# koide3/hdl_graph_slam

Hardware: AMD Instinct MI355X
Metric: registrations/sec (64-beam ~120k-pt pair), loop-closure batch (higher is better)
Workload: dtype f64; 1 GPU; loop-closure batch: 64 candidate keyframes/GPU x HDL-64E (~118849 pts) vs 1 query keyframe, FAST_GICP + getFitnessScore, cold (index + covariances rebuilt every step); candidate set: SURVEY 8d (distinct ray-casts at poses within 20 m of the query, guess = ground truth + 0.5 m / 2 deg noise, z forced to 0); candidates_per_gpu=64, points_per_cloud=118849, method=FAST_GICP, distinct_scans=16, parallelism=single GPU

## Files before the change

### hdl_graph_slam_amd/csrc/hgs_bvh.h

```cpp
#pragma once
#include "hgs_math.h"

namespace hgs {

constexpr int kLeaf = 8;

#if defined(__HIPCC__)
typedef float4 Float4;
#else
struct alignas(16) Float4 {
  float x, y, z, w;
};
#endif

struct BvhView {
  const Float4* nodes;
  const Float4* pts;
  const Float4* lpts;
  int P;
  int n;
};

HGS_HD void bvh_load_box(const Float4* nodes, uint32_t n, float* mn, float* mx) {
  const float* g = reinterpret_cast<const float*>(nodes) + 32 * (size_t)(n >> 2) + (n & 3u);
// ... 166 lines not shown
```

### hdl_graph_slam_amd/csrc/hgs_consts.h

```cpp
#pragma once
#include <cfloat>
#include <cmath>

#include "../../include/hgs_registration.h"
#include "hgs_floor.h"
#include "hgs_gicp.h"
#include "hgs_icp.h"
#include "hgs_ndt.h"
#include "hgs_vgicp.h"

namespace hgs {

inline GicpConsts gicp_consts(const hgs_params& p) {
  GicpConsts c;
  const double thr = p.max_correspondence_distance;
  c.max_corr2 = thr * thr;
  c.search_bound2 = c.max_corr2 >= (double)FLT_MAX ? FLT_MAX : nextafterf((float)c.max_corr2, FLT_MAX);
  c.rotation_eps = p.rotation_epsilon;
  c.translation_eps = p.transformation_epsilon;
  c.lm_init_lambda_factor = p.lm_init_lambda_factor;
  c.lm_max_iterations = p.lm_max_iterations;
  c.max_iterations = p.max_iterations;
  c.k_correspondences = p.correspondence_randomness;
  return c;
}

inline VgicpConsts vgicp_consts(const hgs_params& p) {
  VgicpConsts c;
  c.resolution = p.resolution;
  c.search = p.neighbor_search == HGS_DIRECT27 ? 3 : (p.neighbor_search == HGS_DIRECT7 ? 2 : 1);
  c.pad = 0;
  return c;
}

inline IcpConsts icp_consts(const hgs_params& p) {
  IcpConsts c;
  const double thr = p.max_correspondence_distance;
  c.max_corr2 = thr * thr;
  c.search_bound2 = c.max_corr2 >= (double)FLT_MAX ? FLT_MAX : nextafterf((float)c.max_corr2, FLT_MAX);
  c.max_iterations = p.max_iterations;
  c.trans_eps = p.transformation_epsilon;
  c.rot_thr = p.rotation_epsilon > 0 ? p.rotation_epsilon : 1.0 - p.transformation_epsilon;
  c.reciprocal = p.icp_reciprocal ? 1 : 0;
  c.pad = 0;
  return c;
}

inline NdtConsts ndt_consts(const hgs_params& p) {
  NdtConsts c;
  const double c1 = 10.0 * (1 - p.ndt_outlier_ratio);
  const double c2 = p.ndt_outlier_ratio / std::pow(p.resolution, 3);
  const double d3 = -std::log(c2);
  c.gauss_d1 = -std::log(c1 + c2) - d3;
  c.gauss_d2 = -2 * std::log((-std::log(c1 * std::exp(-0.5) + c2) - d3) / c.gauss_d1);
  c.step_size = p.ndt_step_size;
  c.trans_eps = p.transformation_epsilon;
  c.max_iterations = p.max_iterations;
  c.search = p.neighbor_search == HGS_DIRECT1 ? 1 : (p.neighbor_search == HGS_KDTREE ? 0 : 2);
  c.kdtree_radius2 = (float)(p.resolution * p.resolution);
// ... 24 lines not shown
```

### hdl_graph_slam_amd/csrc/hgs_device.h

```cpp
#pragma once
#include <hip/hip_runtime.h>
#include "hgs_gicp.h"
#include "hgs_floor.h"
#include "hgs_icp.h"
#include "hgs_ndt.h"
#include "hgs_vgicp.h"

namespace hgs {

struct CloudMeta {
  int nvalid;
  int ndt_ncells;
  unsigned bbmin[3];
  unsigned bbmax[3];
  int ndt_min_b[3], ndt_max_b[3], ndt_div_mul[3];
  int ndt_error;
  int vg_ncells;
  int vg_min_b[3], vg_max_b[3], vg_div_mul[3];
  int vg_error;
  int pad[1];
};

struct CloudDesc {
  const float4* raw;
// ... 68 lines not shown
void launch_hilbert_keys(hipStream_t s, const CloudDesc* descs, int ncloud, int max_n, unsigned long long* keys, unsigned* vals, int drop_bits);
void launch_gather_sorted(hipStream_t s, const CloudDesc* descs, int ncloud, int max_slots, const unsigned* sorted_vals);
void launch_build_tree(hipStream_t s, const CloudDesc* descs, int ncloud, int max_P);
void launch_knn_cov(hipStream_t s, const CloudDesc* descs, int ncloud, int max_n, int k, int qpw, int reg_method, int gather ,
                    double* raw_stage = nullptr );

void launch_gicp_init(hipStream_t s, GicpState* states, const float* guesses, int B, Progress prog);
struct Guess16 {
  float m[16];
};
void launch_gicp_init1(hipStream_t s, GicpState* states, const float* guess_host , Progress prog);
void launch_gicp_linearize(hipStream_t s, const CloudDesc* descs, TargetView tgt, const GicpState* states, GicpConsts c, double* partials, int max_blocks, int B,
                           int qpw);
void launch_gicp_solve(hipStream_t s, const CloudDesc* descs, GicpState* states, GicpConsts c, const double* partials, int max_blocks, int B,
                       int tile_points );
void launch_gicp_error(hipStream_t s, const CloudDesc* descs, TargetView tgt, const GicpState* states, double* partials_err, int max_blocks, int B);
void launch_gicp_linearize_round2(hipStream_t s, const CloudDesc* descs, TargetView tgt, const GicpState* states_in, GicpState* states_out, GicpConsts c, double* partials,
                                  const double* partials_err, int max_blocks , int lin_blocks , int B, int qpw, Progress prog,
                                  DevResult* results, DevResult* early_out );
void launch_gicp_error_round2(hipStream_t s, const CloudDesc* descs, TargetView tgt, const GicpState* states_in, GicpState* states_out, GicpConsts c, const double* partials,
                              double* partials_err, int max_blocks, int err_blocks , int B, int lin_tile_points);
void launch_gicp_decide(hipStream_t s, const CloudDesc* descs, GicpState* states, GicpConsts c, const double* partials_err, int max_blocks, int B, Progress prog);
void launch_gicp_results(hipStream_t s, const GicpState* states, DevResult* out, int B);

void launch_icp_init(hipStream_t s, IcpState* states, const float* guesses, int B, Progress prog);
void launch_icp_correspond(hipStream_t s, const CloudDesc* descs, TargetView tgt, const IcpState* states, IcpConsts c, double* partials, int max_blocks, int B);
void launch_icp_solve(hipStream_t s, const CloudDesc* descs, IcpState* states, IcpConsts c, const double* partials, int max_blocks, int B, Progress prog);
void launch_icp_results(hipStream_t s, const IcpState* states, DevResult* out, int B);

void launch_fitness(hipStream_t s, const CloudDesc* descs, TargetView tgt, const DevResult* poses, double max_range, double* partials, int max_blocks, int B,
                    int use_seed, int qpw);
void launch_fitness_final(hipStream_t s, const CloudDesc* descs, const double* partials, int max_blocks, DevResult* out, int B, int tile_pts);
void launch_gicp_linearize(hipStream_t s, const CloudDesc* descs, const TargetView* tviews, const GicpState* states, GicpConsts c, double* partials, int max_blocks, int B,
                           int qpw);
void launch_gicp_error(hipStream_t s, const CloudDesc* descs, const TargetView* tviews, const GicpState* states, double* partials_err, int max_blocks, int B);
void launch_gicp_linearize_round2(hipStream_t s, const CloudDesc* descs, const TargetView* tviews, const GicpState* states_in, GicpState* states_out, GicpConsts c, double* partials,
                                  const double* partials_err, int max_blocks, int lin_blocks, int B, int qpw, Progress prog, DevResult* results, DevResult* early_out);
void launch_gicp_error_round2(hipStream_t s, const CloudDesc* descs, const TargetView* tviews, const GicpState* states_in, GicpState* states_out, GicpConsts c, const double* partials,
                              double* partials_err, int max_blocks, int err_blocks, int B, int lin_tile_points);
void launch_icp_correspond(hipStream_t s, const CloudDesc* descs, const TargetView* tviews, const IcpState* states, IcpConsts c, double* partials, int max_blocks, int B);
void launch_fitness(hipStream_t s, const CloudDesc* descs, const TargetView* tviews, const DevResult* poses, double max_range, double* partials, int max_blocks, int B,
                    int use_seed, int qpw);
}
struct hgs_result;
namespace hgs {
void launch_results_to_records(hipStream_t s, const DevResult* res, const int* candidate_ids, int n, int n_slots, ::hgs_result* out);
void launch_nn_query(hipStream_t s, TargetView tgt, const float4* q, int nq, int* idx, float* d2);
void launch_seed_grid_build(hipStream_t s, const float4* pts, const CloudMeta* meta, int n_max, unsigned* tab, int bits);
inline size_t seed_grid_entries(int bits) { return ((size_t)1 << bits) + ((size_t)1 << (bits - 2)) + ((size_t)1 << (bits - 4)); }
void launch_transform(hipStream_t s, const float4* raw, int n, const float* T16_colmajor_dev, float4* out);
// ... 90 lines not shown
```

### hdl_graph_slam_amd/csrc/hgs_engine.hip

```cpp
#include <hip/hip_runtime.h>
#include <algorithm>
#include <atomic>
#include <chrono>
#include <climits>
#include <condition_variable>
#include <cmath>
#include <cstdio>
#include <cstdlib>
#include <cstring>
#include <exception>
#include <limits>
#include <mutex>
#include <new>
#include <stdexcept>
#include <string>
#include <thread>
#include <vector>

#include "../../include/hgs_registration.h"
#include "hgs_comm.h"
#include "hgs_consts.h"
#include "hgs_device.h"
#include "hgs_resources.h"
#include "hgs_sort.h"
// ... 67 lines not shown
  int prefilter_fast = 1;
  int upload_trace = 0;
  int floor_chunk = 64;
  int early_run_ahead = 2;
  int early_result = 1;
  PinnedBuffer h_early;
  hipEvent_t early_event = nullptr;
  bool early_pending = false, early_valid = false;
  int fused_rounds = 1;
  int fused_rounds_below = 262144;
  int fused_rounds_max_problems = kFusedRoundMaxProblems, fused_rounds_max_blocks = 640;
  int cov_split = 1;
  int resident_descs = 1;
  int knn_qpw_tiny = -1;
  int knn_tiny_below = 32768;
  int seed_grid = 1;
  int knn_replay = -1;
  int batch_lanes = 0;
  std::string err;
  hgs_cloud* target = nullptr;
  hgs_cloud* source = nullptr;
  bool own_target = false, own_source = false;
  float final_T[16];

  DeviceBuffer staging, sort_keys[2], sort_vals[2], sort_tmp, descs, states, angles, partials, partials_err, results, guesses, done, misc;
  DeviceBuffer lane_partials[7], lane_partials_err[7];
  DeviceBuffer ndt_accum;
  DeviceBuffer group_tviews, group_corr;
  hgs::Comm* comm = nullptr;
  DeviceBuffer comm_send, comm_recv, comm_ids;
// ... 637 lines not shown
  return upload_descs(h, sources, false, &s.d_descs, nullptr, corr_of);
}

bool corr_seeds_fitness(int method) { return method == HGS_FAST_GICP || method == HGS_ICP; }
void lane_fitness(hgs_handle* h, BatchLane& L, const BatchShape& s, double max_range, bool corr_seeds) {
  StageTimer tm(h, HGS_STAGE_FITNESS);
  DevResult* res = h->results.as<DevResult>() + L.b0;
  with_lane_target(s, L, s.d_tviews ? TargetView{} : target_view(h->target),
                   [&](auto tgt) { launch_fitness(L.stream, s.d_descs + L.b0, tgt, res, max_range, L.partials_err, s.max_blocks, L.B, corr_seeds ? 1 : 0, s.qpw); });
  launch_fitness_final(L.stream, s.d_descs + L.b0, L.partials_err, s.max_blocks, res, L.B, s.nn_tile);
}
void lane_fitness_tail(hgs_handle* h, BatchLane& L, const BatchShape& s, const double* fit_max_range) {
  if (fit_max_range) lane_fitness(h, L, s, *fit_max_range, corr_seeds_fitness(h->prm.method));
}

int run_gicp_rounds(hgs_handle* h, const BatchShape& s, const float* guesses_host, bool guess_in_args, const double* fit_max_range) {
  const int B = s.B, max_blocks = s.max_blocks;
  hgs_cloud* tgt = h->target;
  const bool voxel = h->prm.method == HGS_FAST_VGICP;
  const GicpConsts c = gicp_consts(h->prm);
  const VgicpConsts vc = vgicp_consts(h->prm);
  const bool round2 = s.gicp_round2;
  const bool early = round2 && B == 1 && !fit_max_range && h->early_result && !h->profiling;
  DevResult* early_out = nullptr;
  if (early) {
    HGS_HIP(h, h->h_early.reserve(sizeof(DevResult)));
    early_out = h->h_early.as<DevResult>();
  }
  HGS_HIP(h, h->states.reserve((size_t)B * sizeof(GicpState) * (round2 ? 2 : 1)));
  GicpState* st = h->states.as<GicpState>();
  GicpState* st_other = st + B;
  const TargetView tv = s.d_tviews ? TargetView{} : target_view(tgt);
  const NdtTargetView vtv = voxel ? vgicp_target_view(tgt) : NdtTargetView{};
  const long max_rounds = (long)std::max(1, c.max_iterations) * std::max(1, c.lm_max_iterations) + 2 + (round2 ? 1 : 0);
  std::vector<BatchLane> lanes;
// ... 26 lines not shown
      });
      return;
    }
    {
      StageTimer tm(h, HGS_STAGE_LINEARIZE);
      if (voxel) launch_vgicp_linearize(L.stream, dd, vtv, ls, vc, L.partials, max_blocks, L.B);
      else with_lane_target(s, L, tv, [&](auto t) { launch_gicp_linearize(L.stream, dd, t, ls, c, L.partials, max_blocks, L.B, s.qpw); });
    }
    {
      StageTimer tm(h, HGS_STAGE_SOLVE);
      launch_gicp_solve(L.stream, dd, ls, c, L.partials, max_blocks, L.B, voxel ? kBlock : s.nn_tile);
    }
    {
      StageTimer tm(h, HGS_STAGE_ERROR);
      if (voxel) launch_vgicp_error(L.stream, dd, vtv, ls, vc, L.partials_err, max_blocks, L.B);
      else with_lane_target(s, L, tv, [&](auto t) { launch_gicp_error(L.stream, dd, t, ls, L.partials_err, max_blocks, L.B); });
    }
    {
      StageTimer tm(h, HGS_STAGE_SOLVE);
      launch_gicp_decide(L.stream, dd, ls, c, L.partials_err, max_blocks, L.B, L.prog);
    }
  }, finish_lane, early ? (long)h->early_run_ahead : kRunAhead);
  HGS_TRY(close_lanes(h, lanes));
  if (h->early_valid) {
    if (!h->early_event) HGS_HIP(h, hipEventCreateWithFlags(&h->early_event, hipEventDisableTiming));
    HGS_HIP(h, hipEventRecord(h->early_event, h->stream));
    h->early_pending = true;
  }
  return HGS_OK;
}

int run_icp_rounds(hgs_handle* h, const BatchShape& s, const double* fit_max_range) {
  const int B = s.B, max_blocks = s.max_blocks;
  const IcpConsts c = icp_consts(h->prm);
  HGS_HIP(h, h->states.reserve((size_t)B * sizeof(IcpState)));
  IcpState* st = h->states.as<IcpState>();
  const TargetView tv = s.d_tviews ? TargetView{} : target_view(h->target);
  const long max_rounds = (long)std::max(0, c.max_iterations) + 2;
  std::vector<BatchLane> lanes;
  HGS_TRY(open_lanes(h, B, (size_t)max_blocks * kAccIcp * sizeof(double), (size_t)max_blocks * 2 * sizeof(double), lanes, s.err_blocks));
  auto finish_lane = [&](BatchLane& L) {
    launch_icp_results(L.stream, st + L.b0, h->results.as<DevResult>() + L.b0, L.B);
    lane_fitness_tail(h, L, s, fit_max_range);
  };
  for (BatchLane& L : lanes) launch_icp_init(L.stream, st + L.b0, h->guesses.as<float>() + (size_t)L.b0 * 16, L.B, L.prog);
  drive_lanes(lanes, max_rounds, [&](BatchLane& L) {
    {
      StageTimer tm(h, HGS_STAGE_LINEARIZE);
      with_lane_target(s, L, tv, [&](auto t) { launch_icp_correspond(L.stream, s.d_descs + L.b0, t, st + L.b0, c, L.partials, max_blocks, L.B); });
// ... 274 lines not shown
  const std::string k(key);
  if (k == "batch_lanes") h->batch_lanes = value <= 0 ? 0 : std::min(kMaxLanes, value);
  else if (k == "lane_start") h->lane_start = value != 0 ? 1 : 0;
  else if (k == "ndt_sort") h->ndt_sort = std::max(-1, std::min(1, value));
  else if (k == "cov_split") h->cov_split = value != 0 ? 1 : 0;
  else if (k == "fused_rounds") h->fused_rounds = value != 0 ? 1 : 0;
  else if (k == "early_result") h->early_result = value != 0 ? 1 : 0;
  else if (k == "early_run_ahead") h->early_run_ahead = std::max(1, std::min(8, value));
  else if (k == "fused_rounds_max_problems") h->fused_rounds_max_problems = std::max(0, value);
  else if (k == "fused_rounds_max_blocks") h->fused_rounds_max_blocks = std::max(0, value);
  else if (k == "fused_rounds_below") h->fused_rounds_below = std::max(0, value);
  else if (k == "resident_descs") h->resident_descs = value != 0 ? 1 : 0;
  else if (k == "knn_qpw_tiny") h->knn_qpw_tiny = value < 0 ? -1 : std::max(0, std::min(32, value & ~7));
  else if (k == "knn_tiny_below") h->knn_tiny_below = std::max(0, value);
  else if (k == "seed_grid") h->seed_grid = value != 0 ? 1 : 0;
  else if (k == "knn_replay") h->knn_replay = std::max(-1, std::min(2, value));
  else if (k == "ndt_resident") h->ndt_resident_blocks = std::max(0, value);
  else if (k == "ndt_chunk") h->ndt_chunk = std::max(0, value);
  else if (k == "hilbert_levels") h->hilbert_levels = std::max(4, std::min(16, value));
  else if (k == "nn_qpw") h->nn_qpw = value == 16 ? 16 : (value == 32 ? 32 : (value == 64 ? 64 : 0));
  else if (k == "nn_qpw16_below") h->nn_qpw16_below = std::max(0, value);
  else if (k == "nn_qpw32_below") h->nn_qpw32_below = std::max(0, value);
  else if (k == "upload_trace") h->upload_trace = value != 0 ? 1 : 0;
  else if (k == "prefilter_fast") h->prefilter_fast = value != 0 ? 1 : 0;
  else if (k == "floor_chunk") h->floor_chunk = std::max(1, std::min(kFloorMaxChunk, value));
  else {
    h->err = "hgs_debug_set_option: unknown option '" + k + "'";
    return HGS_ERR_INVALID_ARGUMENT;
  }
  return HGS_OK;
// ... 1278 lines not shown
  const bool voxel = h->prm.method == HGS_FAST_VGICP;
  std::vector<hgs_cloud*> all{s, t};
  HGS_TRY(ensure_cov(h, all, h->prm.correspondence_randomness));
  if (voxel) HGS_TRY(ensure_vgicp_target(h, t));
  const int max_blocks = std::max(1, ((int)s->n_input + kBlock - 1) / kBlock);
  std::vector<hgs_cloud*> src{s};
  const CloudDesc* d_descs = nullptr;
  HGS_TRY(upload_descs(h, src, false, &d_descs, nullptr));
  HGS_HIP(h, h->states.reserve(sizeof(GicpState)));
  HGS_HIP(h, h->partials.reserve((size_t)max_blocks * kAcc * sizeof(double)));
  HGS_HIP(h, h->misc.reserve(64 * sizeof(double)));
  HGS_HIP(h, hipMemsetAsync(h->partials.p, 0, (size_t)max_blocks * kAcc * sizeof(double), h->stream));
  HGS_HIP(h, hipMemcpyAsync(h->misc.p, T12, 12 * sizeof(double), hipMemcpyHostToDevice, h->stream));
  launch_gicp_debug_state(h->stream, h->states.as<GicpState>(), h->misc.as<double>());
  if (voxel) launch_vgicp_linearize(h->stream, d_descs, vgicp_target_view(t), h->states.as<GicpState>(), vgicp_consts(h->prm), h->partials.as<double>(), max_blocks, 1);
  else launch_gicp_linearize(h->stream, d_descs, target_view(t), h->states.as<GicpState>(), gicp_consts(h->prm), h->partials.as<double>(), max_blocks, 1, 64);
  double* d_out = h->misc.as<double>() + 16;
  launch_reduce_partials(h->stream, h->partials.as<double>(), max_blocks, kAcc, d_out);
  double acc[kAcc];
  HGS_HIP(h, hipMemcpyAsync(acc, d_out, sizeof(acc), hipMemcpyDeviceToHost, h->stream));
  const size_t s_slots = (size_t)s->P * kLeaf, t_slots = (size_t)t->P * kLeaf;
  std::vector<float4> spts, tpts;
  std::vector<int> dcorr;
  int s_nvalid = 0;
  if (corr) {
    spts.resize(s_slots), tpts.resize(t_slots), dcorr.resize(s_slots);
    HGS_HIP(h, hipMemcpyAsync(spts.data(), s->desc.pts, s_slots * sizeof(float4), hipMemcpyDeviceToHost, h->stream));
    HGS_HIP(h, hipMemcpyAsync(tpts.data(), t->desc.pts, t_slots * sizeof(float4), hipMemcpyDeviceToHost, h->stream));
    HGS_HIP(h, hipMemcpyAsync(dcorr.data(), s->desc.corr, s_slots * sizeof(int), hipMemcpyDeviceToHost, h->stream));
    HGS_HIP(h, hipMemcpyAsync(&s_nvalid, &s->desc.meta->nvalid, sizeof(int), hipMemcpyDeviceToHost, h->stream));
  }
// ... 27 lines not shown
  if (!h->source) return HGS_ERR_NO_SOURCE;
  HGS_TRY(set_device(h));
  hgs_cloud *s = h->source, *t = h->target;
  std::vector<hgs_cloud*> all{s, t};
  HGS_TRY(ensure_index(h, all));
  const int max_blocks = std::max(1, ((int)s->n_input + kTileNN - 1) / kTileNN);
  std::vector<hgs_cloud*> src{s};
  const CloudDesc* d_descs = nullptr;
  HGS_TRY(upload_descs(h, src, false, &d_descs, nullptr));
  IcpState st;
  for (int i = 0; i < 12; i++) st.x.m[i] = T12[i];
  st.mse = st.mse_prev = DBL_MAX, st.phase = ICP_RUN, st.iterations = st.passes = st.converged = 0;
  HGS_HIP(h, h->states.reserve(sizeof(IcpState)));
  HGS_HIP(h, h->partials.reserve((size_t)max_blocks * kAccIcp * sizeof(double)));
  HGS_HIP(h, hipMemcpyAsync(h->states.p, &st, sizeof(st), hipMemcpyHostToDevice, h->stream));
  launch_icp_correspond(h->stream, d_descs, target_view(t), h->states.as<IcpState>(), icp_consts(h->prm), h->partials.as<double>(), max_blocks, 1);
  HGS_HIP(h, hipGetLastError());
  std::vector<double> part((size_t)max_blocks * kAccIcp);
  int s_nvalid = 0;
  HGS_HIP(h, hipMemcpyAsync(&s_nvalid, &s->desc.meta->nvalid, sizeof(int), hipMemcpyDeviceToHost, h->stream));
  HGS_HIP(h, hipMemcpyAsync(part.data(), h->partials.p, part.size() * sizeof(double), hipMemcpyDeviceToHost, h->stream));
  const size_t s_slots = (size_t)s->P * kLeaf, t_slots = (size_t)t->P * kLeaf;
  std::vector<float4> spts, tpts;
  std::vector<int> dcorr;
  if (corr) {
    spts.resize(s_slots), tpts.resize(t_slots), dcorr.resize(s_slots);
    HGS_HIP(h, hipMemcpyAsync(spts.data(), s->desc.pts, s_slots * sizeof(float4), hipMemcpyDeviceToHost, h->stream));
    HGS_HIP(h, hipMemcpyAsync(tpts.data(), t->desc.pts, t_slots * sizeof(float4), hipMemcpyDeviceToHost, h->stream));
    HGS_HIP(h, hipMemcpyAsync(dcorr.data(), s->desc.corr, s_slots * sizeof(int), hipMemcpyDeviceToHost, h->stream));
  }
  HGS_HIP(h, hipStreamSynchronize(h->stream));
// ... 137 lines not shown
```

### hdl_graph_slam_amd/csrc/hgs_gicp.h

```cpp
#pragma once
#include "hgs_bvh.h"

namespace hgs {

constexpr int kAcc = 28;

struct GicpConsts {
  double max_corr2;
  float search_bound2;
  double rotation_eps, translation_eps;
  double lm_init_lambda_factor;
  int lm_max_iterations;
  int max_iterations;
  int k_correspondences;
};

HGS_HD Sym3 gicp_neighbour_cov(const double* s1, const Sym3& s2, int found, int k, double lambda) {
  const double inv_f = 1.0 / (double)found, inv_k = 1.0 / (double)k;
  const double mx = s1[0] * inv_f, my = s1[1] * inv_f, mz = s1[2] * inv_f;
  Sym3 c;
  c.xx = (s2.xx - found * mx * mx) * inv_k + lambda;
  c.xy = (s2.xy - found * mx * my) * inv_k;
  c.xz = (s2.xz - found * mx * mz) * inv_k;
  c.yy = (s2.yy - found * my * my) * inv_k + lambda;
  c.yz = (s2.yz - found * my * mz) * inv_k;
  c.zz = (s2.zz - found * mz * mz) * inv_k + lambda;
  return c;
}
HGS_HD Sym3 gicp_regularized_cov(const double* s1, const Sym3& s2, int found, int k) {
// ... 252 lines not shown
```

### hdl_graph_slam_amd/csrc/hgs_icp.h

```cpp
#pragma once
#include "hgs_math.h"

namespace hgs {

constexpr int kAccIcp = 17;

struct IcpConsts {
  double max_corr2;
  float search_bound2;
  int max_iterations;
  double trans_eps;
  double rot_thr;
  int reciprocal;
  int pad;
};

enum IcpPhase { ICP_RUN = 0, ICP_DONE = 2 };

struct IcpState {
  Pose x;
  double mse;
  double mse_prev;
  int phase;
  int iterations;
  int passes;
  int converged;
};

HGS_HD void icp_state_init(IcpState& s, const float* guess_colmajor) {
// ... 148 lines not shown
```

### hdl_graph_slam_amd/csrc/hgs_kernels.hip

```cpp
#include <hip/hip_runtime.h>
#include "../../include/hgs_registration.h"
#include "hgs_device.h"
#include "hgs_wave_bvh.h"

namespace hgs {

#ifndef HGS_OPAQUE_POINTER
#define HGS_OPAQUE_POINTER(p) asm volatile("" : "+v"(p))
#define HGS_WAIT_VMEM() asm volatile("s_waitcnt vmcnt(0)" ::: "memory")
#define HGS_LANE_ID(dst) asm volatile("v_mbcnt_lo_u32_b32 %0, -1, 0\n\tv_mbcnt_hi_u32_b32 %0, -1, %0" : "=v"(dst))
#endif
#ifndef HGS_COMPILER_MEMORY_BARRIER
#define HGS_COMPILER_MEMORY_BARRIER() asm volatile("" ::: "memory")
#endif
#ifndef HGS_LOAD_GLOBAL_XYZ
__device__ __forceinline__ float4 hgs_load_global_xyz(const float4* p) {
  const __attribute__((address_space(1))) float* g = (const __attribute__((address_space(1))) float*)(p);
  return make_float4(g[0], g[1], g[2], 0.f);
}
#define HGS_LOAD_GLOBAL_XYZ(p) hgs_load_global_xyz(p)
#define HGS_OPAQUE_OFFSET(off) asm volatile("" : "+v"(off))
#define HGS_WAIT_VMEM_TRACKED() __builtin_amdgcn_s_waitcnt(0x0F70)
#endif
#ifndef HGS_LINEARIZE_WAVES
// ... 287 lines not shown
}
void launch_hilbert_keys(hipStream_t s, const CloudDesc* descs, int ncloud, int max_n, unsigned long long* keys, unsigned* vals, int drop_bits) {
  if (max_n <= 0) return;
  hipLaunchKernelGGL(k_hilbert_keys, dim3((max_n + kBlock - 1) / kBlock, ncloud), dim3(kBlock), 0, s, descs, keys, vals, drop_bits);
}

__global__ __launch_bounds__(kBlock) void k_gather_sorted(const CloudDesc* descs, const unsigned* __restrict__ sorted_vals) {
  const CloudDesc d = descs[blockIdx.y];
  const int i = blockIdx.x * kBlock + threadIdx.x;
  if (i >= d.P * kLeaf) return;
  float4 p = make_float4(INFINITY, INFINITY, INFINITY, __int_as_float(-1));
  if (i < d.meta->nvalid) p = d.raw[sorted_vals[d.sort_off + i]];
  d.pts[i] = p;
  float* leaf = reinterpret_cast<float*>(d.lpts) + 32 * (size_t)(i >> 3) + (i & 7);
  leaf[0] = p.x, leaf[8] = p.y, leaf[16] = p.z, leaf[24] = p.w;
  if (d.pad) d.corr[i] = -1;
}
void launch_gather_sorted(hipStream_t s, const CloudDesc* descs, int ncloud, int max_slots, const unsigned* sorted_vals) {
  if (max_slots <= 0) return;
  hipLaunchKernelGGL(k_gather_sorted, dim3((max_slots + kBlock - 1) / kBlock, ncloud), dim3(kBlock), 0, s, descs, sorted_vals);
}

__device__ __forceinline__ void store_walk_sentinels(float4* nodes) {
  const float mn[3] = {INFINITY, INFINITY, INFINITY}, mx[3] = {-INFINITY, -INFINITY, -INFINITY};
  bvh_store_box(nodes, 0u, mn, mx);
  bvh_store_box(nodes, 1u, mn, mx);
}

__global__ __launch_bounds__(kBlock) void k_build_bottom(const CloudDesc* descs) {
  const CloudDesc d = descs[blockIdx.y];
  const int P = d.P;
// ... 356 lines not shown
  const unsigned n = (unsigned)t.meta->nvalid;
  int best = -1;
  float best_d = FLT_MAX;
  const unsigned e[3] = {e0, e1, e2};
#pragma unroll
  for (int l = 0; l < 3; l++) {
    if (e[l] < n) {
      const float4 p = t.pts[e[l]];
      const float d = dist2f(q, p.x, p.y, p.z);
      if (d < best_d) best_d = d, best = (int)e[l];
    }
  }
  return best;
}

__device__ __forceinline__ void packet_nn1(const BvhView& tv, float* park, const F3& q, bool active, float bound2, int seed, int qpw, float& d2, int& pos, int& orig) {
  const bool seeded = seed >= 0 && seed < tv.n;
  int leaf;
  bool tie, found;
  if (__ballot(active && !seeded) != 0ull) wave_nn1_quad<true, true>(tv, park, q, active, bound2, seed, qpw >> 1, d2, leaf, tie, found);
  else wave_nn1_quad<false, true>(tv, park, q, active, bound2, seed, qpw >> 1, d2, leaf, tie, found);
  if (__ballot(tie) != 0ull) {
    const F3 qa[1] = {q};
    const bool aa[1] = {active};
    const int sa[1] = {seed};
    float da[1];
    int pa[1], oa[1];
    wave_nn1<1>(tv, park, qa, aa, bound2, sa, da, pa, oa, qpw);
    d2 = da[0], pos = pa[0], orig = oa[0];
  } else {
    nn1_resolve_leaf(tv, q, found ? leaf : -1, d2, pos, orig);
  }
// ... 27 lines not shown
  {
    double t[kAcc];
    gicp_point_terms_by_slot(r, M, t);
#pragma unroll
    for (int j = 0; j < 14; j++) even[j] = t[2 * j];
  }
  __builtin_amdgcn_sched_barrier(0);
  {
    double t[kAcc];
    gicp_point_terms_by_slot(r, M, t);
#pragma unroll
    for (int j = 0; j < 14; j++) odd[j] = t[2 * j + 1];
  }
  wave_sums28_to(even, odd, row, lane);
}

template <bool ROUND2, bool SHORT = false, typename TGT = TargetView>
__global__ __launch_bounds__(kBlock) __attribute__((amdgpu_waves_per_eu(ROUND2 ? 4 : HGS_LINEARIZE_WAVES))) void k_gicp_linearize(const CloudDesc* descs, TGT tgt_arg, const GicpState* states, GicpConsts c,
                                                           double* __restrict__ partials, int max_blocks, int qpw, GicpState* states_out,
                                                           const double* __restrict__ partials_err, Progress prog, DevResult* results, DevResult* early_out) {
  const int b = blockIdx.y;
  const TargetView& tgt = problem_target(tgt_arg, b);
  __shared__ GicpState st2;
  __shared__ double ws2[kGicpControlWorkspace];
  if constexpr (!ROUND2) {
    if (states[b].phase != GICP_LINEARIZE) return;
  }
  const CloudDesc d = descs[b];
  const int n = d.meta->nvalid;
  if constexpr (ROUND2) {
// ... 29 lines not shown
  if (tile >= ntiles) return;
  __shared__ double lds[4 * kAcc];
  __shared__ unsigned arrivals;
  __shared__ __attribute__((aligned(512))) float park[kBlock / 64][kParkFloats];
  if (threadIdx.x == 0) arrivals = 0u;
  __syncthreads();
  const int wave = __builtin_amdgcn_readfirstlane((int)(threadIdx.x >> 6));
  const Pose T = ROUND2 ? st2.x0 : states[b].x0;
  float Tf[12];
  pose_to_float(T, Tf);
  static_assert(kNW == 1, "one packet of 64 consecutive source points per wave");
  const int idx = tile * tile_pts + wave * qpw + (int)(threadIdx.x & 63);
  const bool active = (int)(threadIdx.x & 63) < qpw && idx < n;
  const float4 a = active ? load_stream(d.pts + idx) : make_float4(0.f, 0.f, 0.f, 0.f);
  const F3 q = transform_point_f(Tf, a.x, a.y, a.z);
  const int seed = active ? __builtin_nontemporal_load(d.corr + idx) : -1;
  float d2;
  int j, orig;
  packet_nn1(view_of(tgt), park[wave], q, active, c.search_bound2, seed, qpw, d2, j, orig);
  const double R[9] = {T.m[0], T.m[1], T.m[2], T.m[4], T.m[5], T.m[6], T.m[8], T.m[9], T.m[10]};
  int jj = active ? j : -1;
  if (jj >= 0 && !((double)d2 < c.max_corr2)) jj = -1;
  if (active) __builtin_nontemporal_store(jj, d.corr + idx);
  if constexpr (SHORT) {
    static_assert(ROUND2, "the short-packet form belongs to the two-launch rounds");
    {
      __shared__ int chunk_corr[kBlock];
      int lane;
      HGS_LANE_ID(lane);
      if (lane < qpw) chunk_corr[wave * qpw + lane] = jj;
      unsigned ticket = 0;
      if (lane == 0) ticket = __hip_atomic_fetch_add(&arrivals, 1u, __ATOMIC_ACQ_REL, __HIP_MEMORY_SCOPE_WORKGROUP);
      ticket = (unsigned)__builtin_amdgcn_readlane((int)ticket, 0);
      if (ticket != kBlock / 64 - 1) return;
      const int chunks = tile_pts / 64;
      for (int ch = 0; ch < chunks; ch++) {
        const int i2 = tile * tile_pts + ch * 64 + lane;
        if (tile * tile_pts + ch * 64 >= n) break;
        const int j2 = i2 < n ? chunk_corr[ch * 64 + lane] : -1;
        Sym3 M2 = {0.0, 0.0, 0.0, 0.0, 0.0, 0.0};
        GicpPointResidual r2 = {0.0, 0.0, 0.0, 0.0, 0.0, 0.0, 0.0};
        if (j2 >= 0) {
          const float4 a2 = load_stream(d.pts + i2);
          M2 = gicp_mahalanobis(R, load_cov_stream(d.cov, i2), load_cov(tgt.cov, j2));
          const float4 bp = tgt.pts[j2];
          r2 = gicp_point_residual(T, M2, a2.x, a2.y, a2.z, bp.x, bp.y, bp.z);
        }
        gicp_wave_row(r2, M2, lds, lane);
        __builtin_amdgcn_wave_barrier();
        if (lane < kAcc) partials[((size_t)b * max_blocks + (size_t)tile * chunks + ch) * kAcc + lane] = lds[lane];
        __builtin_amdgcn_wave_barrier();
      }
      return;
    }
  } else {
  Sym3 M = {0.0, 0.0, 0.0, 0.0, 0.0, 0.0};
  GicpPointResidual r = {0.0, 0.0, 0.0, 0.0, 0.0, 0.0, 0.0};
  if (jj >= 0) {
    M = gicp_mahalanobis(R, load_cov_stream(d.cov, idx), load_cov(tgt.cov, jj));
    const float4 bp = tgt.pts[jj];
    r = gicp_point_residual(T, M, a.x, a.y, a.z, bp.x, bp.y, bp.z);
  }
  int lane;
  HGS_LANE_ID(lane);
  double* row = lds + wave * kAcc;
  gicp_wave_row(r, M, row, lane);
  last_wave_stores<kAcc>(lds, &arrivals, partials + ((size_t)b * max_blocks + tile) * kAcc, lane);
  }
}
void launch_gicp_linearize(hipStream_t s, const CloudDesc* descs, TargetView tgt, const GicpState* states, GicpConsts c, double* partials,
// ... 70 lines not shown
      const bool chunked = lin_tile_points < kBlock;
      const int ntiles_lin = chunked ? (n + kBlock - 1) / kBlock : (n + lin_tile_points - 1) / lin_tile_points;
      reduce_tiles<kAcc>(partials + (size_t)b * max_blocks * kAcc, ntiles_lin, acc2, scratch2, chunked ? (n + 63) / 64 : 0);
      if (threadIdx.x == 0) gicp_after_linearize(st2, acc2, c, ws2);
    }
    __syncthreads();
    if (blockIdx.x == 0) gicp_state_store(states_out + b, st2);
    if (st2.phase != GICP_TRY) return;
  }
  const int ntiles = (n + kBlock - 1) / kBlock;
  if ((int)blockIdx.x >= ntiles) return;
  const int tile = (int)blockIdx.x;
  const int i = tile * kBlock + threadIdx.x;
  __shared__ double lds[4];
  double err = 0.0;
  if (i < n) {
    const int j = d.corr[i];
    if (j >= 0) {
      const Pose T0 = ROUND2 ? st2.x0 : states[b].x0;
      const Pose Ti = ROUND2 ? st2.xi : states[b].xi;
      const double R[9] = {T0.m[0], T0.m[1], T0.m[2], T0.m[4], T0.m[5], T0.m[6], T0.m[8], T0.m[9], T0.m[10]};
      const Sym3 M = gicp_mahalanobis(R, load_cov(d.cov, i), load_cov(tgt.cov, j));
      const float4 a = d.pts[i], bp = tgt.pts[j];
      err = gicp_point_terms<false>(Ti, M, a.x, a.y, a.z, bp.x, bp.y, bp.z, nullptr);
    }
  }
  block_reduce_store<1>(&err, partials_err + (size_t)b * max_blocks + tile, lds);
}
void launch_gicp_error(hipStream_t s, const CloudDesc* descs, TargetView tgt, const GicpState* states, double* partials_err, int max_blocks, int B) {
  hipLaunchKernelGGL(k_gicp_error<false>, dim3(max_blocks, B), dim3(kBlock), 0, s, descs, tgt, states, partials_err, max_blocks, GicpConsts{}, (GicpState*)nullptr, (const double*)nullptr, 0);
}
void launch_gicp_error_round2(hipStream_t s, const CloudDesc* descs, TargetView tgt, const GicpState* states_in, GicpState* states_out, GicpConsts c, const double* partials,
                              double* partials_err, int max_blocks, int err_blocks, int B, int lin_tile_points) {
  hipLaunchKernelGGL(k_gicp_error<true>, dim3(err_blocks, B), dim3(kBlock), 0, s, descs, tgt, states_in, partials_err, max_blocks, c, states_out, partials, lin_tile_points);
}
void launch_gicp_error(hipStream_t s, const CloudDesc* descs, const TargetView* tviews, const GicpState* states, double* partials_err, int max_blocks, int B) {
  hipLaunchKernelGGL((k_gicp_error<false, const TargetView*>), dim3(max_blocks, B), dim3(kBlock), 0, s, descs, tviews, states, partials_err, max_blocks, GicpConsts{}, (GicpState*)nullptr,
                     (const double*)nullptr, 0);
}
void launch_gicp_error_round2(hipStream_t s, const CloudDesc* descs, const TargetView* tviews, const GicpState* states_in, GicpState* states_out, GicpConsts c, const double* partials,
                              double* partials_err, int max_blocks, int err_blocks, int B, int lin_tile_points) {
  hipLaunchKernelGGL((k_gicp_error<true, const TargetView*>), dim3(err_blocks, B), dim3(kBlock), 0, s, descs, tviews, states_in, partials_err, max_blocks, c, states_out, partials, lin_tile_points);
}

__device__ __forceinline__ bool gicp_decide_wave(int ntiles, GicpState* state, const GicpConsts& c, const double* __restrict__ problem_partials_err) {
  __shared__ GicpState st;
  __shared__ double ws[kGicpControlWorkspace];
  bool finished_now = false;
  double s = 0;
  if (threadIdx.x < 64) {
    for (int k = threadIdx.x; k < (int)(sizeof(GicpState) / sizeof(double)); k += 64) reinterpret_cast<double*>(&st)[k] = reinterpret_cast<const double*>(state)[k];
    for (int t = threadIdx.x; t < ntiles; t += 64) s += problem_partials_err[t];
// ... 56 lines not shown
  const int ntiles = (n + kTileNN - 1) / kTileNN;
  const int tile = xcd_tile(blockIdx.x, ntiles);
  if (tile >= ntiles) return;
  __shared__ double lds[4 * kAccIcp];
  __shared__ unsigned arrivals;
  __shared__ __attribute__((aligned(512))) float park[kBlock / 64][kParkFloats];
  if (threadIdx.x == 0) arrivals = 0u;
  __syncthreads();
  const int wave = __builtin_amdgcn_readfirstlane((int)(threadIdx.x >> 6));
  const Pose T = states[b].x;
  static_assert(kNW == 1 && kTileNN == (kBlock / 64) * qpw, "one packet of 64 consecutive source points per wave");
  const int idx = tile * kTileNN + wave * qpw + (int)(threadIdx.x & 63);
  const bool active = idx < n;
  const float4 a = active ? load_stream(d.pts + idx) : make_float4(0.f, 0.f, 0.f, 0.f);
  const F3 q = icp_move_point(T, a.x, a.y, a.z);
  const int seed = active ? __builtin_nontemporal_load(d.corr + idx) : -1;
  float d2;
  int j, orig;
  packet_nn1(view_of(tgt), park[wave], q, active, c.search_bound2, seed, qpw, d2, j, orig);
  int jj = active ? j : -1;
  if (jj >= 0 && !((double)d2 <= c.max_corr2)) jj = -1;
  const float4 bp = jj >= 0 ? tgt.pts[jj] : make_float4(0.f, 0.f, 0.f, 0.f);
  if constexpr (RECIPROCAL) {
    const bool ractive = jj >= 0;
    if (__ballot(ractive) != 0ull) {
      const F3 r = icp_unmove_point(T, bp.x, bp.y, bp.z);
      BvhView sv;
      sv.nodes = d.nodes, sv.pts = d.pts, sv.lpts = d.lpts, sv.P = d.P, sv.n = n;
      float rd2;
      int rj, rorig;
      packet_nn1(sv, park[wave], r, ractive, c.search_bound2, ractive ? idx : -1, qpw, rd2, rj, rorig);
      if (ractive && !(rj >= 0 && rorig == __float_as_int(a.w) && (double)rd2 <= c.max_corr2)) jj = -1;
    }
  }
  if (active) __builtin_nontemporal_store(jj, d.corr + idx);
  double acc[kAccIcp];
  if (jj >= 0) {
    icp_pair_terms(q, bp.x, bp.y, bp.z, d2, acc);
  } else {
#pragma unroll
    for (int k = 0; k < kAccIcp; k++) acc[k] = 0.0;
  }
  int lane;
  HGS_LANE_ID(lane);
  int slot[kAccIcp];
#pragma unroll
  for (int k = 0; k < kAccIcp; k++) slot[k] = k;
  wave_sums_to<kAccIcp>(acc, slot, lds + wave * kAccIcp, lane);
  last_wave_stores<kAccIcp>(lds, &arrivals, partials + ((size_t)b * max_blocks + tile) * kAccIcp, lane);
}
// ... 1536 lines not shown
```

Before: 5379 registrations/sec.

## Mark unmatched correspondences and skip empty waves in GICP/ICP kernels

```diff
diff --git a/hdl_graph_slam_amd/csrc/hgs_bvh.h b/hdl_graph_slam_amd/csrc/hgs_bvh.h
--- a/hdl_graph_slam_amd/csrc/hgs_bvh.h
+++ b/hdl_graph_slam_amd/csrc/hgs_bvh.h
@@ -4,6 +4,11 @@
 namespace hgs {
 
 constexpr int kLeaf = 8;
+
+constexpr int kCorrStale = -1;
+constexpr int kCorrNone = -2;
+constexpr int kCorrFlagOrderedOnUnmatched = 1;
+constexpr int kCorrFlagNoEmptyWaveExit = 2;
 
 #if defined(__HIPCC__)
 typedef float4 Float4;
diff --git a/hdl_graph_slam_amd/csrc/hgs_consts.h b/hdl_graph_slam_amd/csrc/hgs_consts.h
--- a/hdl_graph_slam_amd/csrc/hgs_consts.h
+++ b/hdl_graph_slam_amd/csrc/hgs_consts.h
@@ -22,6 +22,7 @@
   c.lm_max_iterations = p.lm_max_iterations;
   c.max_iterations = p.max_iterations;
   c.k_correspondences = p.correspondence_randomness;
+  c.flags = 0;
   return c;
 }
 
@@ -42,7 +43,7 @@
   c.trans_eps = p.transformation_epsilon;
   c.rot_thr = p.rotation_epsilon > 0 ? p.rotation_epsilon : 1.0 - p.transformation_epsilon;
   c.reciprocal = p.icp_reciprocal ? 1 : 0;
-  c.pad = 0;
+  c.flags = 0;
   return c;
 }
 
diff --git a/hdl_graph_slam_amd/csrc/hgs_device.h b/hdl_graph_slam_amd/csrc/hgs_device.h
--- a/hdl_graph_slam_amd/csrc/hgs_device.h
+++ b/hdl_graph_slam_amd/csrc/hgs_device.h
@@ -106,7 +106,7 @@
                            int qpw);
 void launch_gicp_solve(hipStream_t s, const CloudDesc* descs, GicpState* states, GicpConsts c, const double* partials, int max_blocks, int B,
                        int tile_points );
-void launch_gicp_error(hipStream_t s, const CloudDesc* descs, TargetView tgt, const GicpState* states, double* partials_err, int max_blocks, int B);
+void launch_gicp_error(hipStream_t s, const CloudDesc* descs, TargetView tgt, const GicpState* states, double* partials_err, int max_blocks, int B, int flags );
 void launch_gicp_linearize_round2(hipStream_t s, const CloudDesc* descs, TargetView tgt, const GicpState* states_in, GicpState* states_out, GicpConsts c, double* partials,
                                   const double* partials_err, int max_blocks , int lin_blocks , int B, int qpw, Progress prog,
                                   DevResult* results, DevResult* early_out );
@@ -125,7 +125,7 @@
 void launch_fitness_final(hipStream_t s, const CloudDesc* descs, const double* partials, int max_blocks, DevResult* out, int B, int tile_pts);
 void launch_gicp_linearize(hipStream_t s, const CloudDesc* descs, const TargetView* tviews, const GicpState* states, GicpConsts c, double* partials, int max_blocks, int B,
                            int qpw);
-void launch_gicp_error(hipStream_t s, const CloudDesc* descs, const TargetView* tviews, const GicpState* states, double* partials_err, int max_blocks, int B);
+void launch_gicp_error(hipStream_t s, const CloudDesc* descs, const TargetView* tviews, const GicpState* states, double* partials_err, int max_blocks, int B, int flags);
 void launch_gicp_linearize_round2(hipStream_t s, const CloudDesc* descs, const TargetView* tviews, const GicpState* states_in, GicpState* states_out, GicpConsts c, double* partials,
                                   const double* partials_err, int max_blocks, int lin_blocks, int B, int qpw, Progress prog, DevResult* results, DevResult* early_out);
 void launch_gicp_error_round2(hipStream_t s, const CloudDesc* descs, const TargetView* tviews, const GicpState* states_in, GicpState* states_out, GicpConsts c, const double* partials,
diff --git a/hdl_graph_slam_amd/csrc/hgs_engine.hip b/hdl_graph_slam_amd/csrc/hgs_engine.hip
--- a/hdl_graph_slam_amd/csrc/hgs_engine.hip
+++ b/hdl_graph_slam_amd/csrc/hgs_engine.hip
@@ -105,6 +105,8 @@
   int resident_descs = 1;
   int knn_qpw_tiny = -1;
   int knn_tiny_below = 32768;
+  int ordered_on_unmatched = 0;
+  int empty_wave_exit = 1;
   int seed_grid = 1;
   int knn_replay = -1;
   int batch_lanes = 0;
@@ -772,11 +774,23 @@
   if (fit_max_range) lane_fitness(h, L, s, *fit_max_range, corr_seeds_fitness(h->prm.method));
 }
 
+int corr_flags(const hgs_handle* h) { return (h->ordered_on_unmatched ? kCorrFlagOrderedOnUnmatched : 0) | (h->empty_wave_exit ? 0 : kCorrFlagNoEmptyWaveExit); }
+GicpConsts engine_gicp_consts(const hgs_handle* h) {
+  GicpConsts c = gicp_consts(h->prm);
+  c.flags = corr_flags(h);
+  return c;
+}
+IcpConsts engine_icp_consts(const hgs_handle* h) {
+  IcpConsts c = icp_consts(h->prm);
+  c.flags = corr_flags(h);
+  return c;
+}
+
 int run_gicp_rounds(hgs_handle* h, const BatchShape& s, const float* guesses_host, bool guess_in_args, const double* fit_max_range) {
   const int B = s.B, max_blocks = s.max_blocks;
   hgs_cloud* tgt = h->target;
   const bool voxel = h->prm.method == HGS_FAST_VGICP;
-  const GicpConsts c = gicp_consts(h->prm);
+  const GicpConsts c = engine_gicp_consts(h);
   const VgicpConsts vc = vgicp_consts(h->prm);
   const bool round2 = s.gicp_round2;
   const bool early = round2 && B == 1 && !fit_max_range && h->early_result && !h->profiling;
@@ -833,7 +847,7 @@
     {
       StageTimer tm(h, HGS_STAGE_ERROR);
       if (voxel) launch_vgicp_error(L.stream, dd, vtv, ls, vc, L.partials_err, max_blocks, L.B);
-      else with_lane_target(s, L, tv, [&](auto t) { launch_gicp_error(L.stream, dd, t, ls, L.partials_err, max_blocks, L.B); });
+      else with_lane_target(s, L, tv, [&](auto t) { launch_gicp_error(L.stream, dd, t, ls, L.partials_err, max_blocks, L.B, c.flags); });
     }
     {
       StageTimer tm(h, HGS_STAGE_SOLVE);
@@ -851,7 +865,7 @@
 
 int run_icp_rounds(hgs_handle* h, const BatchShape& s, const double* fit_max_range) {
   const int B = s.B, max_blocks = s.max_blocks;
-  const IcpConsts c = icp_consts(h->prm);
+  const IcpConsts c = engine_icp_consts(h);
   HGS_HIP(h, h->states.reserve((size_t)B * sizeof(IcpState)));
   IcpState* st = h->states.as<IcpState>();
   const TargetView tv = s.d_tviews ? TargetView{} : target_view(h->target);
@@ -1156,6 +1170,8 @@
   else if (k == "knn_qpw_tiny") h->knn_qpw_tiny = value < 0 ? -1 : std::max(0, std::min(32, value & ~7));
   else if (k == "knn_tiny_below") h->knn_tiny_below = std::max(0, value);
   else if (k == "seed_grid") h->seed_grid = value != 0 ? 1 : 0;
+  else if (k == "ordered_on_unmatched") h->ordered_on_unmatched = value != 0 ? 1 : 0;
+  else if (k == "empty_wave_exit") h->empty_wave_exit = value != 0 ? 1 : 0;
   else if (k == "knn_replay") h->knn_replay = std::max(-1, std::min(2, value));
   else if (k == "ndt_resident") h->ndt_resident_blocks = std::max(0, value);
   else if (k == "ndt_chunk") h->ndt_chunk = std::max(0, value);
@@ -2464,7 +2480,7 @@
   HGS_HIP(h, hipMemcpyAsync(h->misc.p, T12, 12 * sizeof(double), hipMemcpyHostToDevice, h->stream));
   launch_gicp_debug_state(h->stream, h->states.as<GicpState>(), h->misc.as<double>());
   if (voxel) launch_vgicp_linearize(h->stream, d_descs, vgicp_target_view(t), h->states.as<GicpState>(), vgicp_consts(h->prm), h->partials.as<double>(), max_blocks, 1);
-  else launch_gicp_linearize(h->stream, d_descs, target_view(t), h->states.as<GicpState>(), gicp_consts(h->prm), h->partials.as<double>(), max_blocks, 1, 64);
+  else launch_gicp_linearize(h->stream, d_descs, target_view(t), h->states.as<GicpState>(), engine_gicp_consts(h), h->partials.as<double>(), max_blocks, 1, 64);
   double* d_out = h->misc.as<double>() + 16;
   launch_reduce_partials(h->stream, h->partials.as<double>(), max_blocks, kAcc, d_out);
   double acc[kAcc];
@@ -2522,7 +2538,7 @@
   HGS_HIP(h, h->states.reserve(sizeof(IcpState)));
   HGS_HIP(h, h->partials.reserve((size_t)max_blocks * kAccIcp * sizeof(double)));
   HGS_HIP(h, hipMemcpyAsync(h->states.p, &st, sizeof(st), hipMemcpyHostToDevice, h->stream));
-  launch_icp_correspond(h->stream, d_descs, target_view(t), h->states.as<IcpState>(), icp_consts(h->prm), h->partials.as<double>(), max_blocks, 1);
+  launch_icp_correspond(h->stream, d_descs, target_view(t), h->states.as<IcpState>(), engine_icp_consts(h), h->partials.as<double>(), max_blocks, 1);
   HGS_HIP(h, hipGetLastError());
   std::vector<double> part((size_t)max_blocks * kAccIcp);
   int s_nvalid = 0;
diff --git a/hdl_graph_slam_amd/csrc/hgs_gicp.h b/hdl_graph_slam_amd/csrc/hgs_gicp.h
--- a/hdl_graph_slam_amd/csrc/hgs_gicp.h
+++ b/hdl_graph_slam_amd/csrc/hgs_gicp.h
@@ -13,6 +13,7 @@
   int lm_max_iterations;
   int max_iterations;
   int k_correspondences;
+  int flags;
 };
 
 HGS_HD Sym3 gicp_neighbour_cov(const double* s1, const Sym3& s2, int found, int k, double lambda) {
diff --git a/hdl_graph_slam_amd/csrc/hgs_icp.h b/hdl_graph_slam_amd/csrc/hgs_icp.h
--- a/hdl_graph_slam_amd/csrc/hgs_icp.h
+++ b/hdl_graph_slam_amd/csrc/hgs_icp.h
@@ -12,7 +12,7 @@
   double trans_eps;
   double rot_thr;
   int reciprocal;
-  int pad;
+  int flags;
 };
 
 enum IcpPhase { ICP_RUN = 0, ICP_DONE = 2 };
diff --git a/hdl_graph_slam_amd/csrc/hgs_kernels.hip b/hdl_graph_slam_amd/csrc/hgs_kernels.hip
--- a/hdl_graph_slam_amd/csrc/hgs_kernels.hip
+++ b/hdl_graph_slam_amd/csrc/hgs_kernels.hip
@@ -325,7 +325,7 @@
   d.pts[i] = p;
   float* leaf = reinterpret_cast<float*>(d.lpts) + 32 * (size_t)(i >> 3) + (i & 7);
   leaf[0] = p.x, leaf[8] = p.y, leaf[16] = p.z, leaf[24] = p.w;
-  if (d.pad) d.corr[i] = -1;
+  if (d.pad) d.corr[i] = kCorrStale;
 }
 void launch_gather_sorted(hipStream_t s, const CloudDesc* descs, int ncloud, int max_slots, const unsigned* sorted_vals) {
   if (max_slots <= 0) return;
@@ -712,8 +712,9 @@
   return best;
 }
 
-__device__ __forceinline__ void packet_nn1(const BvhView& tv, float* park, const F3& q, bool active, float bound2, int seed, int qpw, float& d2, int& pos, int& orig) {
-  const bool seeded = seed >= 0 && seed < tv.n;
+__device__ __forceinline__ void packet_nn1(const BvhView& tv, float* park, const F3& q, bool active, float bound2, int seed, int qpw, float& d2, int& pos, int& orig,
+                                           int flags = 0) {
+  const bool seeded = (seed >= 0 && seed < tv.n) || (seed == kCorrNone && !(flags & kCorrFlagOrderedOnUnmatched));
   int leaf;
   bool tie, found;
   if (__ballot(active && !seeded) != 0ull) wave_nn1_quad<true, true>(tv, park, q, active, bound2, seed, qpw >> 1, d2, leaf, tie, found);
@@ -771,6 +772,7 @@
   }
   wave_sums28_to(even, odd, row, lane);
 }
+__device__ __forceinline__ double gicp_empty_row_value(int slot) { return ((0x7007738u >> slot) & 1u) ? -0.0 : 0.0; }
 
 template <bool ROUND2, bool SHORT = false, typename TGT = TargetView>
 __global__ __launch_bounds__(kBlock) __attribute__((amdgpu_waves_per_eu(ROUND2 ? 4 : HGS_LINEARIZE_WAVES))) void k_gicp_linearize(const CloudDesc* descs, TGT tgt_arg, const GicpState* states, GicpConsts c,
@@ -830,14 +832,15 @@
   const bool active = (int)(threadIdx.x & 63) < qpw && idx < n;
   const float4 a = active ? load_stream(d.pts + idx) : make_float4(0.f, 0.f, 0.f, 0.f);
   const F3 q = transform_point_f(Tf, a.x, a.y, a.z);
-  const int seed = active ? __builtin_nontemporal_load(d.corr + idx) : -1;
+  const int seed = active ? __builtin_nontemporal_load(d.corr + idx) : kCorrStale;
   float d2;
   int j, orig;
-  packet_nn1(view_of(tgt), park[wave], q, active, c.search_bound2, seed, qpw, d2, j, orig);
+  packet_nn1(view_of(tgt), park[wave], q, active, c.search_bound2, seed, qpw, d2, j, orig, c.flags);
   const double R[9] = {T.m[0], T.m[1], T.m[2], T.m[4], T.m[5], T.m[6], T.m[8], T.m[9], T.m[10]};
   int jj = active ? j : -1;
   if (jj >= 0 && !((double)d2 < c.max_corr2)) jj = -1;
-  if (active) __builtin_nontemporal_store(jj, d.corr + idx);
+  if (active) __builtin_nontemporal_store(jj >= 0 ? jj : kCorrNone, d.corr + idx);
+  const bool empty_exit = !(c.flags & kCorrFlagNoEmptyWaveExit);
   if constexpr (SHORT) {
     static_assert(ROUND2, "the short-packet form belongs to the two-launch rounds");
     {
@@ -854,6 +857,10 @@
         const int i2 = tile * tile_pts + ch * 64 + lane;
         if (tile * tile_pts + ch * 64 >= n) break;
         const int j2 = i2 < n ? chunk_corr[ch * 64 + lane] : -1;
+        if (empty_exit && __ballot(j2 >= 0) == 0ull) {
+          if (lane < kAcc) partials[((size_t)b * max_blocks + (size_t)tile * chunks + ch) * kAcc + lane] = gicp_empty_row_value(lane);
+          continue;
+        }
         Sym3 M2 = {0.0, 0.0, 0.0, 0.0, 0.0, 0.0};
         GicpPointResidual r2 = {0.0, 0.0, 0.0, 0.0, 0.0, 0.0, 0.0};
         if (j2 >= 0) {
@@ -870,6 +877,13 @@
       return;
     }
   } else {
+  if (empty_exit && __ballot(jj >= 0) == 0ull) {
+    int lane;
+    HGS_LANE_ID(lane);
+    if (lane < kAcc) lds[wave * kAcc + lane] = gicp_empty_row_value(lane);
+    last_wave_stores<kAcc>(lds, &arrivals, partials + ((size_t)b * max_blocks + tile) * kAcc, lane);
+    return;
+  }
   Sym3 M = {0.0, 0.0, 0.0, 0.0, 0.0, 0.0};
   GicpPointResidual r = {0.0, 0.0, 0.0, 0.0, 0.0, 0.0, 0.0};
   if (jj >= 0) {
@@ -970,8 +984,8 @@
   const int i = tile * kBlock + threadIdx.x;
   __shared__ double lds[4];
   double err = 0.0;
-  if (i < n) {
-    const int j = d.corr[i];
+  const int j = i < n ? d.corr[i] : -1;
+  if ((c.flags & kCorrFlagNoEmptyWaveExit) || __ballot(j >= 0) != 0ull) {
     if (j >= 0) {
       const Pose T0 = ROUND2 ? st2.x0 : states[b].x0;
       const Pose Ti = ROUND2 ? st2.xi : states[b].xi;
@@ -980,18 +994,26 @@
       const float4 a = d.pts[i], bp = tgt.pts[j];
       err = gicp_point_terms<false>(Ti, M, a.x, a.y, a.z, bp.x, bp.y, bp.z, nullptr);
     }
-  }
-  block_reduce_store<1>(&err, partials_err + (size_t)b * max_blocks + tile, lds);
-}
-void launch_gicp_error(hipStream_t s, const CloudDesc* descs, TargetView tgt, const GicpState* states, double* partials_err, int max_blocks, int B) {
-  hipLaunchKernelGGL(k_gicp_error<false>, dim3(max_blocks, B), dim3(kBlock), 0, s, descs, tgt, states, partials_err, max_blocks, GicpConsts{}, (GicpState*)nullptr, (const double*)nullptr, 0);
+    err = wave_sum(err);
+  }
+  if ((threadIdx.x & 63) == 0) lds[threadIdx.x >> 6] = err;
+  __syncthreads();
+  if (threadIdx.x == 0) partials_err[(size_t)b * max_blocks + tile] = (lds[0] + lds[1]) + (lds[2] + lds[3]);
+}
+static GicpConsts gicp_error_consts(int flags) {
+  GicpConsts c{};
+  c.flags = flags;
+  return c;
+}
+void launch_gicp_error(hipStream_t s, const CloudDesc* descs, TargetView tgt, const GicpState* states, double* partials_err, int max_blocks, int B, int flags) {
+  hipLaunchKernelGGL(k_gicp_error<false>, dim3(max_blocks, B), dim3(kBlock), 0, s, descs, tgt, states, partials_err, max_blocks, gicp_error_consts(flags), (GicpState*)nullptr, (const double*)nullptr, 0);
 }
 void launch_gicp_error_round2(hipStream_t s, const CloudDesc* descs, TargetView tgt, const GicpState* states_in, GicpState* states_out, GicpConsts c, const double* partials,
                               double* partials_err, int max_blocks, int err_blocks, int B, int lin_tile_points) {
   hipLaunchKernelGGL(k_gicp_error<true>, dim3(err_blocks, B), dim3(kBlock), 0, s, descs, tgt, states_in, partials_err, max_blocks, c, states_out, partials, lin_tile_points);
 }
-void launch_gicp_error(hipStream_t s, const CloudDesc* descs, const TargetView* tviews, const GicpState* states, double* partials_err, int max_blocks, int B) {
-  hipLaunchKernelGGL((k_gicp_error<false, const TargetView*>), dim3(max_blocks, B), dim3(kBlock), 0, s, descs, tviews, states, partials_err, max_blocks, GicpConsts{}, (GicpState*)nullptr,
+void launch_gicp_error(hipStream_t s, const CloudDesc* descs, const TargetView* tviews, const GicpState* states, double* partials_err, int max_blocks, int B, int flags) {
+  hipLaunchKernelGGL((k_gicp_error<false, const TargetView*>), dim3(max_blocks, B), dim3(kBlock), 0, s, descs, tviews, states, partials_err, max_blocks, gicp_error_consts(flags), (GicpState*)nullptr,
                      (const double*)nullptr, 0);
 }
 void launch_gicp_error_round2(hipStream_t s, const CloudDesc* descs, const TargetView* tviews, const GicpState* states_in, GicpState* states_out, GicpConsts c, const double* partials,
@@ -1078,12 +1100,13 @@
   const bool active = idx < n;
   const float4 a = active ? load_stream(d.pts + idx) : make_float4(0.f, 0.f, 0.f, 0.f);
   const F3 q = icp_move_point(T, a.x, a.y, a.z);
-  const int seed = active ? __builtin_nontemporal_load(d.corr + idx) : -1;
+  const int seed = active ? __builtin_nontemporal_load(d.corr + idx) : kCorrStale;
   float d2;
   int j, orig;
-  packet_nn1(view_of(tgt), park[wave], q, active, c.search_bound2, seed, qpw, d2, j, orig);
+  packet_nn1(view_of(tgt), park[wave], q, active, c.search_bound2, seed, qpw, d2, j, orig, c.flags);
   int jj = active ? j : -1;
   if (jj >= 0 && !((double)d2 <= c.max_corr2)) jj = -1;
+  const bool none = jj < 0;
   const float4 bp = jj >= 0 ? tgt.pts[jj] : make_float4(0.f, 0.f, 0.f, 0.f);
   if constexpr (RECIPROCAL) {
     const bool ractive = jj >= 0;
@@ -1093,11 +1116,18 @@
       sv.nodes = d.nodes, sv.pts = d.pts, sv.lpts = d.lpts, sv.P = d.P, sv.n = n;
       float rd2;
       int rj, rorig;
-      packet_nn1(sv, park[wave], r, ractive, c.search_bound2, ractive ? idx : -1, qpw, rd2, rj, rorig);
+      packet_nn1(sv, park[wave], r, ractive, c.search_bound2, ractive ? idx : -1, qpw, rd2, rj, rorig, c.flags);
       if (ractive && !(rj >= 0 && rorig == __float_as_int(a.w) && (double)rd2 <= c.max_corr2)) jj = -1;
     }
   }
-  if (active) __builtin_nontemporal_store(jj, d.corr + idx);
+  if (active) __builtin_nontemporal_store(none ? kCorrNone : jj, d.corr + idx);
+  if (!(c.flags & kCorrFlagNoEmptyWaveExit) && __ballot(jj >= 0) == 0ull) {
+    int lane;
+    HGS_LANE_ID(lane);
+    if (lane < kAccIcp) lds[wave * kAccIcp + lane] = 0.0;
+    last_wave_stores<kAccIcp>(lds, &arrivals, partials + ((size_t)b * max_blocks + tile) * kAccIcp, lane);
+    return;
+  }
   double acc[kAccIcp];
   if (jj >= 0) {
     icp_pair_terms(q, bp.x, bp.y, bp.z, d2, acc);
```

New measurement: 5361 registrations/sec. Within noise of the previous version (-0.3%).
